# arkworks-rs/pcd

Hardware: NVIDIA B200
Metric: pcd_step_proofs_per_sec (higher is better)
Workload: dtype u32 (10x32-bit limbs, Montgomery, integer only)

## Files before the change

### pcd_b200/csrc/fp.cuh

```cuda
#pragma once
#include "constants.cuh"

#define FP_LIMBS 10

#if defined(__CUDACC__)
static __constant__ u32 pcd_modc_r4[FP_LIMBS + 2] = {
    ParamsR4::mod(0), ParamsR4::mod(1), ParamsR4::mod(2), ParamsR4::mod(3), ParamsR4::mod(4), ParamsR4::mod(5),
    ParamsR4::mod(6), ParamsR4::mod(7), ParamsR4::mod(8), ParamsR4::mod(9), ParamsR4::INV, 0};
#endif
template <class P>
PCD_HD u32 fp_mod_opaque(int i) {
#if defined(__CUDA_ARCH__)
  if (P::ID == 0) return pcd_modc_r4[i];
#endif
  return i < FP_LIMBS ? P::mod(i) : P::INV;
}

template <class P>
struct Fp {
  u32 l[FP_LIMBS];
  typedef P Params;
  static constexpr int WORDS = FP_LIMBS;

  PCD_HD static Fp zero() {
    Fp r;
#pragma unroll
    for (int i = 0; i < FP_LIMBS; i++) r.l[i] = 0;
    return r;
  }
  PCD_HD static Fp one() {
    Fp r;
#pragma unroll
    for (int i = 0; i < FP_LIMBS; i++) r.l[i] = P::one(i);
    return r;
  }
  PCD_HD static Fp r2() {
    Fp r;
#pragma unroll
    for (int i = 0; i < FP_LIMBS; i++) r.l[i] = P::r2(i);
    return r;
  }
  PCD_HD bool is_zero() const {
    u32 t = 0;
#pragma unroll
    for (int i = 0; i < FP_LIMBS; i++) t |= l[i];
    return t == 0;
  }
  PCD_HD bool operator==(const Fp& o) const {
    u32 t = 0;
#pragma unroll
    for (int i = 0; i < FP_LIMBS; i++) t |= l[i] ^ o.l[i];
    return t == 0;
  }
  PCD_HD bool operator!=(const Fp& o) const { return !(*this == o); }

  PCD_HD static void reduce_once(u32* a) {
    u32 t[FP_LIMBS];
    t[0] = prims::sub_cc(a[0], P::mod(0));
#pragma unroll
    for (int i = 1; i < FP_LIMBS; i++) t[i] = prims::subc_cc(a[i], P::mod(i));
    u32 borrow = prims::subc(0, 0);
#pragma unroll
    for (int i = 0; i < FP_LIMBS; i++) a[i] = borrow ? a[i] : t[i];
  }

  PCD_HD friend Fp operator+(const Fp& a, const Fp& b) {
    Fp r;
    r.l[0] = prims::add_cc(a.l[0], b.l[0]);
#pragma unroll
    for (int i = 1; i < FP_LIMBS - 1; i++) r.l[i] = prims::addc_cc(a.l[i], b.l[i]);
    r.l[FP_LIMBS - 1] = prims::addc(a.l[FP_LIMBS - 1], b.l[FP_LIMBS - 1]);
    reduce_once(r.l);
    return r;
  }
  PCD_HD friend Fp operator-(const Fp& a, const Fp& b) {
    Fp r;
    r.l[0] = prims::sub_cc(a.l[0], b.l[0]);
#pragma unroll
    for (int i = 1; i < FP_LIMBS; i++) r.l[i] = prims::subc_cc(a.l[i], b.l[i]);
    u32 borrow = prims::subc(0, 0);
    u32 t[FP_LIMBS];
    t[0] = prims::add_cc(r.l[0], P::mod(0));
#pragma unroll
    for (int i = 1; i < FP_LIMBS - 1; i++) t[i] = prims::addc_cc(r.l[i], P::mod(i));
    t[FP_LIMBS - 1] = prims::addc(r.l[FP_LIMBS - 1], P::mod(FP_LIMBS - 1));
#pragma unroll
    for (int i = 0; i < FP_LIMBS; i++) r.l[i] = borrow ? t[i] : r.l[i];
    return r;
  }
  PCD_HD Fp neg() const {
    if (is_zero()) return *this;
    Fp r;
    r.l[0] = prims::sub_cc(P::mod(0), l[0]);
#pragma unroll
    for (int i = 1; i < FP_LIMBS - 1; i++) r.l[i] = prims::subc_cc(P::mod(i), l[i]);
    r.l[FP_LIMBS - 1] = prims::subc(P::mod(FP_LIMBS - 1), l[FP_LIMBS - 1]);
    return r;
  }
  PCD_HD Fp dbl() const { return *this + *this; }

  PCD_HD static void mul_n(u32* acc, const u32* a, u32 bi, int n = FP_LIMBS) {
#pragma unroll
    for (int j = 0; j < n; j += 2) {
      acc[j] = prims::mul_lo(a[j], bi);
      acc[j + 1] = prims::mul_hi(a[j], bi);
    }
  }
  PCD_HD static void cmad_n(u32* acc, const u32* a, u32 bi, int n = FP_LIMBS) {
    acc[0] = prims::mad_lo_cc(a[0], bi, acc[0]);
    acc[1] = prims::madc_hi_cc(a[0], bi, acc[1]);
#pragma unroll
    for (int j = 2; j < n; j += 2) {
      acc[j] = prims::madc_lo_cc(a[j], bi, acc[j]);
      acc[j + 1] = prims::madc_hi_cc(a[j], bi, acc[j + 1]);
    }
  }
  template <int OFF>
  PCD_HD static void cmad_mod(u32* acc, u32 m) {
    acc[0] = prims::mad_lo_cc(fp_mod_opaque<P>(OFF), m, acc[0]);
    acc[1] = prims::madc_hi_cc(fp_mod_opaque<P>(OFF), m, acc[1]);
#pragma unroll
    for (int j = 2; j < FP_LIMBS; j += 2) {
      acc[j] = prims::madc_lo_cc(fp_mod_opaque<P>(OFF + j), m, acc[j]);
      acc[j + 1] = prims::madc_hi_cc(fp_mod_opaque<P>(OFF + j), m, acc[j + 1]);
    }
  }
  PCD_HD static void madc_n_rshift(u32* odd, const u32* a, u32 bi) {
#pragma unroll
    for (int j = 0; j < FP_LIMBS - 2; j += 2) {
      odd[j] = prims::madc_lo_cc(a[j], bi, odd[j + 2]);
      odd[j + 1] = prims::madc_hi_cc(a[j], bi, odd[j + 3]);
    }
    odd[FP_LIMBS - 2] = prims::madc_lo_cc(a[FP_LIMBS - 2], bi, 0);
    odd[FP_LIMBS - 1] = prims::madc_hi(a[FP_LIMBS - 2], bi, 0);
  }
  PCD_HD static void mont_row(u32* even, u32* odd, const u32* a, u32 bi, bool first) {
    if (first) {
      mul_n(odd, a + 1, bi);
      mul_n(even, a, bi);
    } else {
      even[0] = prims::add_cc(even[0], odd[1]);
      madc_n_rshift(odd, a + 1, bi);
      cmad_n(even, a, bi);
      odd[FP_LIMBS - 1] = prims::addc(odd[FP_LIMBS - 1], 0);
    }
    u32 m = prims::mul_lo(even[0], fp_mod_opaque<P>(FP_LIMBS));
    cmad_mod<1>(odd, m);
    cmad_mod<0>(even, m);
    odd[FP_LIMBS - 1] = prims::addc(odd[FP_LIMBS - 1], 0);
  }

  PCD_HD friend Fp operator*(const Fp& a, const Fp& b) {
    return mul_cc(a, b);
  }
  PCD_HD static Fp mul_cc(const Fp& a, const Fp& b) {
    u32 even[FP_LIMBS], odd[FP_LIMBS];
#pragma unroll
    for (int i = 0; i < FP_LIMBS; i += 2) {
      mont_row(even, odd, a.l, b.l[i], i == 0);
      mont_row(odd, even, a.l, b.l[i + 1], false);
    }
    Fp r;
    r.l[0] = prims::add_cc(even[0], odd[1]);
#pragma unroll
    for (int i = 1; i < FP_LIMBS - 1; i++) r.l[i] = prims::addc_cc(even[i], odd[i + 1]);
    r.l[FP_LIMBS - 1] = prims::addc(even[FP_LIMBS - 1], 0);
    reduce_once(r.l);
    return r;
  }
  PCD_HD Fp sqr() const { return (*this) * (*this); }
  PCD_NOINLINE static Fp mul_ni(Fp a, Fp b) { return a * b; }

  template <u32 K>
  PCD_HD Fp mul_small() const {
    static_assert(K >= 1 && K < 256, "small constant");
    Fp acc = *this;
    bool started = false;
    Fp r = *this;
#pragma unroll
    for (int bit = 7; bit >= 0; bit--) {
      if (started) r = r.dbl();
      if ((K >> bit) & 1) {
        if (started) r = r + acc;
        else started = true;
      }
    }
    return r;
  }

  PCD_HD static constexpr u32 pm2(int i) {
    u64 borrow = 2;
    u32 out = 0;
    for (int k = 0; k <= i; k++) {
      u64 v = P::mod(k);
      out = (u32)(v - borrow);
      borrow = (v < borrow) ? 1 : 0;
    }
    return out;
  }
  PCD_HD Fp inverse_fermat() const {
    Fp r = one();
    bool started = false;
    for (int i = FP_LIMBS - 1; i >= 0; i--) {
      u32 e = 0;
#pragma unroll
      for (int k = 0; k < FP_LIMBS; k++)
        if (k == i) e = pm2(k);
      for (int b = 31; b >= 0; b--) {
        if (started) r = r.sqr();
        if ((e >> b) & 1) {
          r = started ? r * (*this) : *this;
          started = true;
        }
      }
    }
    return r;
  }
  PCD_HD static void shr1(u32* a) {
#pragma unroll
    for (int i = 0; i < FP_LIMBS - 1; i++) a[i] = (a[i] >> 1) | (a[i + 1] << 31);
    a[FP_LIMBS - 1] >>= 1;
  }
  PCD_HD static void halve_mod(u32* x) {
    if (x[0] & 1) {
      x[0] = prims::add_cc(x[0], P::mod(0));
#pragma unroll
      for (int i = 1; i < FP_LIMBS - 1; i++) x[i] = prims::addc_cc(x[i], P::mod(i));
      x[FP_LIMBS - 1] = prims::addc(x[FP_LIMBS - 1], P::mod(FP_LIMBS - 1));
    }
    shr1(x);
  }
  PCD_HD static bool geq(const u32* a, const u32* b) {
    prims::sub_cc(a[0], b[0]);
#pragma unroll
    for (int i = 1; i < FP_LIMBS; i++) prims::subc_cc(a[i], b[i]);
    return prims::subc(0, 0) == 0;
  }
  PCD_HD static void sub_raw(u32* a, const u32* b) {
    a[0] = prims::sub_cc(a[0], b[0]);
#pragma unroll
    for (int i = 1; i < FP_LIMBS - 1; i++) a[i] = prims::subc_cc(a[i], b[i]);
    a[FP_LIMBS - 1] = prims::subc(a[FP_LIMBS - 1], b[FP_LIMBS - 1]);
  }
  PCD_HD static bool is_one_raw(const u32* a) {
    u32 t = a[0] ^ 1u;
#pragma unroll
    for (int i = 1; i < FP_LIMBS; i++) t |= a[i];
    return t == 0;
  }
  PCD_HD Fp inverse() const {
    if (is_zero()) return *this;
    u32 u[FP_LIMBS], v[FP_LIMBS];
    Fp x1 = zero(), x2 = zero();
    x1.l[0] = 1;
#pragma unroll
    for (int i = 0; i < FP_LIMBS; i++) {
      u[i] = l[i];
      v[i] = P::mod(i);
    }
    while (!is_one_raw(u) && !is_one_raw(v)) {
      while (!(u[0] & 1)) {
        shr1(u);
        halve_mod(x1.l);
      }
      while (!(v[0] & 1)) {
        shr1(v);
        halve_mod(x2.l);
      }
      if (geq(u, v)) {
        sub_raw(u, v);
        x1 = x1 - x2;
      } else {
        sub_raw(v, u);
        x2 = x2 - x1;
      }
    }
    Fp r = is_one_raw(u) ? x1 : x2;
    return (r * r2()) * r2();
  }
  PCD_HD Fp pow64(u64 e) const {
    Fp r = one();
    Fp base = *this;
    while (e) {
      if (e & 1) r = r * base;
      e >>= 1;
      if (e) base = base.sqr();
    }
    return r;
  }
  PCD_HD Fp from_mont() const {
    Fp o = zero();
    o.l[0] = 1;
    return (*this) * o;
  }
  PCD_HD Fp to_mont() const { return (*this) * r2(); }
  PCD_HD static Fp from_u32(u32 v) {
    Fp o = zero();
    o.l[0] = v;
    return o.to_mont();
  }
  PCD_HD bool lexicographically_largest() const {
    Fp v = from_mont();
    Fp n = neg().from_mont();
#pragma unroll
    for (int i = FP_LIMBS - 1; i >= 0; i--) {
      if (v.l[i] != n.l[i]) return v.l[i] > n.l[i];
    }
    return false;
  }
};

typedef Fp<ParamsR4> FpR4;
typedef Fp<ParamsQ4> FpQ4;
```

### pcd_b200/csrc/msm.cuh

```cuda
#pragma once
#include <cstdlib>

#include <cub/device/device_radix_sort.cuh>
#include <cub/device/device_scan.cuh>

#include "common.cuh"
#include "vecio.cuh"
#include "wec.cuh"

static constexpr int MSM_SCALAR_BITS = 298;
static constexpr int MSM_HEAVY = 1024;
static constexpr int MSM_HEAVY_THREADS = 128;
static constexpr int MSM_MAX_HEAVY = 16384;
static constexpr int MSM_HEAVY_CHUNK = 1024;
static constexpr int MSM_REDUCE_LOGL = 3;
static constexpr int MSM_SUM_PER_GROUP = 4;
static constexpr int MSM_MAX_SPLIT = 4;

__host__ __device__ __forceinline__ int msm_win_start(int j, int c, int nwin, int balanced) {
  if (!balanced) return j * c;
  int base = (MSM_SCALAR_BITS + 1) / nwin, rem = (MSM_SCALAR_BITS + 1) % nwin;
  return j * base + (j < rem ? j : rem);
}

template <class SP>
__global__ void msm_digits_kernel(const u32* __restrict__ scalars, int mont, size_t n_main,
                                  const u32* __restrict__ extra, size_t n, int c, int nwin, int shared,
                                  int* __restrict__ dig, u32* __restrict__ counts, const uint4* __restrict__ bases,
                                  int point_u4, size_t base_first, u32 unit_k) {
  size_t i = (size_t)blockIdx.x * blockDim.x + threadIdx.x;
  if (i >= n) return;
  {
    const uint4* bp = bases + (base_first + i) * (size_t)point_u4;
    u32 any = 0;
    for (int q = 0; q < point_u4; q++) {
      uint4 v = __ldg(bp + q);
      any |= v.x | v.y | v.z | v.w;
    }
    if (any == 0) {
      for (int w = 0; w < nwin; w++) dig[(size_t)w * n + i] = 0;
      return;
    }
  }
  Fp<SP> k;
  const bool is_extra = i >= n_main;
  const uint2* p = reinterpret_cast<const uint2*>(is_extra ? extra + (i - n_main) * 10 : scalars + i * 10);
  if (is_extra) mont = 0;
#pragma unroll
  for (int j = 0; j < 5; j++) {
    uint2 v = __ldg(p + j);
    k.l[2 * j] = v.x;
    k.l[2 * j + 1] = v.y;
  }
  if (mont) k = k.from_mont();
  const u32 B = 1u << (c - 1);
  if (unit_k) {
    u32 rest = 0;
#pragma unroll
    for (int j = 1; j < 10; j++) rest |= k.l[j];
    if (rest == 0 && k.l[0] == 1u) {
      const u32 b = B + (u32)(i & (size_t)(unit_k - 1));
      dig[i] = (int)(b + 1);
      for (int w = 1; w < nwin; w++) dig[(size_t)w * n + i] = 0;
      atomicAdd(&counts[b], 1u);
      return;
    }
  }
  u32 w32[12];
#pragma unroll
  for (int j = 0; j < 10; j++) w32[j] = k.l[j];
  w32[10] = 0;
  w32[11] = 0;
  u32 carry = 0;
  for (int w = 0; w < nwin; w++) {
    int bit = msm_win_start(w, c, nwin, shared);
    int cw = (w + 1 < nwin ? msm_win_start(w + 1, c, nwin, shared) : (shared ? MSM_SCALAR_BITS + 1 : bit + c)) - bit;
    const u32 mask = (1u << cw) - 1;
    const u32 half = 1u << (cw - 1);
    int limb = bit >> 5, off = bit & 31;
    u32 d = 0;
    if (limb < 10) {
      unsigned long long v = w32[limb] | ((unsigned long long)w32[limb + 1] << 32);
      d = (u32)(v >> off) & mask;
    }
    d += carry;
    int sd;
    if (d > half) {
      sd = (int)d - (int)(1u << cw);
      carry = 1;
    } else {
      sd = (int)d;
      carry = 0;
    }
    dig[(size_t)w * n + i] = sd;
    if (sd != 0) {
      u32 b = (u32)(sd < 0 ? -sd : sd) - 1;
      atomicAdd(&counts[(shared ? 0 : (size_t)w * B) + b], 1u);
    }
  }
}

static __global__ void msm_scatter_kernel(const int* __restrict__ dig, size_t n, int c, int nwin, int shared, size_t stride,
                                   size_t offset, u32* __restrict__ cursor, u32* __restrict__ entries) {
  size_t t = (size_t)blockIdx.x * blockDim.x + threadIdx.x;
  if (t >= n * (size_t)nwin) return;
  int sd = dig[t];
  if (sd == 0) return;
  size_t w = t / n, i = t - w * n;
  const u32 B = 1u << (c - 1);
  u32 b = (u32)(sd < 0 ? -sd : sd) - 1;
  u32 pos = atomicAdd(&cursor[(shared ? 0 : w * B) + b], 1u);
  entries[pos] = (u32)(shared ? w * stride + offset + i : i) | (sd < 0 ? 0x80000000u : 0u);
}

static __global__ void msm_sizekey_kernel(const u32* __restrict__ counts, size_t nbuckets, u32* __restrict__ key,
                                          u32* __restrict__ id) {
  size_t g = (size_t)blockIdx.x * blockDim.x + threadIdx.x;
  if (g >= nbuckets) return;
  u32 c = counts[g];
  key[g] = c < 2047u ? c : 2047u;
  id[g] = (u32)g;
}

static __global__ void msm_prof_entries_kernel(const u32* __restrict__ heavy, const u32* __restrict__ offsets, size_t nbuckets,
                                               u32* __restrict__ out) {
  u32 nheavy = heavy[0] < (u32)MSM_MAX_HEAVY ? heavy[0] : (u32)MSM_MAX_HEAVY;
  u32 h = 0;
  for (u32 i = threadIdx.x; i < nheavy; i += 32) h += offsets[heavy[1 + i] + 1] - offsets[heavy[1 + i]];
  for (int d = 16; d > 0; d >>= 1) h += __shfl_xor_sync(0xffffffffu, h, d);
  if (threadIdx.x == 0) {
    out[0] = offsets[nbuckets] - h;
    out[1] = h;
  }
}

__device__ __forceinline__ u32 msm_dynamic_heavy_thr(u32 host_thr, u32 real_total, u32 resident_items, size_t nbuckets,
                                                     u32 split) {
  u32 share = real_total / (resident_items ? resident_items : 1u);
  u32 item = share / 2 > 8u ? share / 2 : 8u;
  u32 dyn = split * item;
  u32 floor_thr = 2u * (u32)(real_total / nbuckets) + 8u;
  if (dyn < floor_thr) dyn = floor_thr;
  if (dyn < 24u) dyn = 24u;
  return dyn < host_thr ? dyn : host_thr;
}

static __global__ void __launch_bounds__(1024) msm_plan_small_kernel(const u32* __restrict__ counts, u32 nbuckets,
                                                                      u32* __restrict__ offsets, u32* __restrict__ cursor,
                                                                      u32* __restrict__ perm, u32* __restrict__ heavy,
                                                                      u32* __restrict__ queue) {
  __shared__ u32 key[1024];
  __shared__ u32 warp_sum[32];
  const u32 t = threadIdx.x;
  const u32 c = t < nbuckets ? counts[t] : 0u;
  key[t] = c < 2047u ? c : 2047u;
  u32 v = c;
  for (int d = 1; d < 32; d <<= 1) {
    u32 o = __shfl_up_sync(0xffffffffu, v, d);
    if ((t & 31u) >= (u32)d) v += o;
  }
  if ((t & 31u) == 31u) warp_sum[t >> 5] = v;
  __syncthreads();
  if (t < 32) {
    u32 w = warp_sum[t];
    for (int d = 1; d < 32; d <<= 1) {
      u32 o = __shfl_up_sync(0xffffffffu, w, d);
      if (t >= (u32)d) w += o;
    }
    warp_sum[t] = w;
  }
  __syncthreads();
  const u32 incl = v + ((t >> 5) ? warp_sum[(t >> 5) - 1] : 0u);
  if (t < nbuckets) {
    offsets[t] = incl - c;
    cursor[t] = incl - c;
    if (t == nbuckets - 1) {
      offsets[nbuckets] = incl;
      cursor[nbuckets] = incl;
    }
    u32 rank = 0;
    const u32 mine = key[t];
    for (u32 j = 0; j < nbuckets; j++) {
      const u32 kj = key[j];
      rank += (kj > mine || (kj == mine && j < t)) ? 1u : 0u;
    }
    perm[rank] = t;
  }
  if (t == 0) {
    heavy[0] = 0;
    queue[0] = 0;
  }
}

template <class C, bool PRE>
__device__ __forceinline__ AffinePoint<typename C::F> ld_base(const void* bases, size_t idx) {
  return ld_vec<AffinePoint<typename C::F>>(bases, idx);
}

template <class C, bool PRE>
__global__ void __launch_bounds__(128) msm_accumulate_kernel(const void* __restrict__ bases,
                                                             const u32* __restrict__ offsets,
                                                             const u32* __restrict__ entries,
                                                             const u32* __restrict__ perm, size_t nbuckets,
                                                             void* __restrict__ buckets, u32* __restrict__ heavy,
                                                             u32* __restrict__ queue, u32 heavy_thr, u32 split,
                                                             u32* __restrict__ hflag, u32 quantum, u32 persistent_from,
                                                             u32 resident_items, u32 nweighted) {
  typedef typename C::F F;
  typedef C CF;
  typedef typename CF::F FF;
  const unsigned lane = threadIdx.x & 31;
  const size_t nitems = nbuckets * split;
  const bool may_retire = blockIdx.x < persistent_from;
  heavy_thr = msm_dynamic_heavy_thr(heavy_thr, offsets[nbuckets], resident_items, nbuckets, split);
  u32 walked = 0;
  for (;;) {
    if (may_retire && __shfl_sync(0xffffffffu, walked, 0) >= quantum) break;
    u32 first = 0;
    if (lane == 0) first = atomicAdd(queue, 32u);
    first = __shfl_sync(0xffffffffu, first, 0);
    if (first >= nitems) break;
    size_t t = (size_t)first + lane;
    if (t >= nitems) continue;
    const u32 part = (u32)(t % split);
    size_t g = perm[t / split];
    u32 lo = offsets[g], hi = offsets[g + 1];
    XYZZ<CF> acc = XYZZ<CF>::inf();
    if (hi - lo > heavy_thr && g < nweighted) {
      if (part != 0) continue;
      u32 slot = atomicAdd(&heavy[0], 1u);
      if (slot < (u32)MSM_MAX_HEAVY) {
        heavy[1 + slot] = (u32)g;
        hflag[g] = 0xffffffffu;
        continue;
      }
      if (split > 1) {
        for (u32 q = 1; q < split; q++) st_vec(buckets, g * split + q, acc);
      }
    } else if (split > 1) {
      const u32 len = hi - lo;
      const u32 a = lo + (u32)(((unsigned long long)len * part) / split);
      hi = lo + (u32)(((unsigned long long)len * (part + 1)) / split);
      lo = a;
    }
    walked += hi - lo;
    for (u32 e = lo; e < hi; e++) {
      u32 ent = entries[e];
      AffinePoint<FF> p = ld_base<C, PRE>(bases, ent & 0x7fffffffu);
      if (ent >> 31) p.y = p.y.neg();
      acc.madd_impl(p);
    }
    st_vec(buckets, g * split + part, acc);
  }
}
template <class CS>
__device__ __forceinline__ AffinePoint<typename CS::F> ld_base_sliced(const void* bases, size_t idx, int l) {
  AffinePoint<typename CS::F> p;
  const char* src = reinterpret_cast<const char*>(bases) + idx * (size_t)240;
  const uint2* px = reinterpret_cast<const uint2*>(src + 40 * l);
  const uint2* py = reinterpret_cast<const uint2*>(src + 120 + 40 * l);
#pragma unroll
  for (int i = 0; i < 5; i++) {
    uint2 a = __ldg(px + i), b = __ldg(py + i);
    p.x.c.l[2 * i] = a.x;
    p.x.c.l[2 * i + 1] = a.y;
    p.y.c.l[2 * i] = b.x;
    p.y.c.l[2 * i + 1] = b.y;
  }
  return p;
}
template <class CS>
__device__ __forceinline__ void st_xyzz_sliced(void* buckets, size_t idx, const XYZZ<CS>& a, int l) {
  char* dst = reinterpret_cast<char*>(buckets) + idx * (size_t)480 + 40 * l;
  const FpR4* co[4] = {&a.x.c, &a.y.c, &a.zz.c, &a.zzz.c};
#pragma unroll
  for (int q = 0; q < 4; q++) {
    uint2* d = reinterpret_cast<uint2*>(dst + 120 * q);
#pragma unroll
    for (int i = 0; i < 5; i++) d[i] = make_uint2(co[q]->l[2 * i], co[q]->l[2 * i + 1]);
  }
}
template <class CS>
__device__ __forceinline__ XYZZ<CS> ld_xyzz_sliced(const void* buckets, size_t idx, int l) {
  XYZZ<CS> a;
  const char* src = reinterpret_cast<const char*>(buckets) + idx * (size_t)480 + 40 * l;
  FpR4* co[4] = {&a.x.c, &a.y.c, &a.zz.c, &a.zzz.c};
#pragma unroll
  for (int q = 0; q < 4; q++) {
    const uint2* d = reinterpret_cast<const uint2*>(src + 120 * q);
#pragma unroll
    for (int i = 0; i < 5; i++) {
      uint2 v = d[i];
      co[q]->l[2 * i] = v.x;
      co[q]->l[2 * i + 1] = v.y;
    }
  }
  return a;
}

#ifndef PCD_SLICED_MIN_CTAS
#define PCD_SLICED_MIN_CTAS 3
#endif
template <class CS, bool PRE>
__global__ void __launch_bounds__(128, PCD_SLICED_MIN_CTAS) msm_accumulate_sliced_kernel(const void* __restrict__ bases,
                                                                    const u32* __restrict__ offsets,
                                                                    const u32* __restrict__ entries,
                                                                    const u32* __restrict__ perm, size_t nbuckets,
                                                                    void* __restrict__ buckets, u32* __restrict__ heavy,
                                                                    u32* __restrict__ queue, u32 heavy_thr, u32 split,
                                                                    u32* __restrict__ hflag, u32 quantum, u32 persistent_from,
                                                             u32 resident_items, u32 nweighted) {
  typedef typename CS::F FF;
  const unsigned lane = threadIdx.x & 31;
  const int l = (int)(lane % 3u);
  const unsigned grp = lane / 3u;
  const size_t nitems = nbuckets * split;
  const bool may_retire = blockIdx.x < persistent_from;
  heavy_thr = msm_dynamic_heavy_thr(heavy_thr, offsets[nbuckets], resident_items, nbuckets, split);
  u32 walked = 0;
  for (;;) {
    if (may_retire && __shfl_sync(0xffffffffu, walked, 0) >= quantum) break;
    u32 first = 0;
    if (lane == 0) first = atomicAdd(queue, 10u);
    first = __shfl_sync(0xffffffffu, first, 0);
    if (first >= nitems) break;
    if (grp >= 10) continue;
    size_t t = (size_t)first + grp;
    if (t >= nitems) continue;
    const u32 part = (u32)(t % split);
    size_t g = perm[t / split];
    u32 lo = offsets[g], hi = offsets[g + 1];
    XYZZ<CS> acc = XYZZ<CS>::inf();
    if (hi - lo > heavy_thr && g < nweighted) {
      if (part != 0) continue;
      u32 slot = 0;
      if (l == 0) slot = atomicAdd(&heavy[0], 1u);
      slot = __shfl_sync(FF::gmask(), slot, (int)(lane - l));
      if (slot < (u32)MSM_MAX_HEAVY) {
        if (l == 0) {
          heavy[1 + slot] = (u32)g;
          hflag[g] = 0xffffffffu;
        }
        continue;
      }
      if (split > 1) {
        for (u32 q = 1; q < split; q++) st_xyzz_sliced<CS>(buckets, g * split + q, acc, l);
      }
    } else if (split > 1) {
      const u32 len = hi - lo;
      const u32 a = lo + (u32)(((unsigned long long)len * part) / split);
      hi = lo + (u32)(((unsigned long long)len * (part + 1)) / split);
      lo = a;
    }
    walked += hi - lo;
    for (u32 e = lo; e < hi; e++) {
      u32 ent = entries[e];
      AffinePoint<FF> p = ld_base_sliced<CS>(bases, ent & 0x7fffffffu, l);
      if (ent >> 31) p.y = p.y.neg();
      acc.madd_impl(p);
    }
    st_xyzz_sliced<CS>(buckets, g * split + part, acc, l);
  }
}
template <class CS>
__global__ void __launch_bounds__(96) msm_fold_parts_sliced_kernel(const void* __restrict__ partials, size_t nbuckets, u32 split,
                                                                   const u32* __restrict__ hflag, void* __restrict__ buckets) {
  const unsigned lane = threadIdx.x & 31, warp = threadIdx.x >> 5;
  if (lane >= 30) return;
  const int l = (int)(lane % 3u);
  size_t g = ((size_t)blockIdx.x * 3 + warp) * 10 + lane / 3u;
  if (g >= nbuckets || hflag[g] == 0xffffffffu) return;
  XYZZ<CS> acc = ld_xyzz_sliced<CS>(partials, g * split, l);
  for (u32 q = 1; q < split; q++) acc.add_impl(ld_xyzz_sliced<CS>(partials, g * split + q, l));
  st_xyzz_sliced<CS>(buckets, g, acc, l);
}

template <class C>
__global__ void __launch_bounds__(128) msm_fold_parts_kernel(const void* __restrict__ partials, size_t nbuckets, u32 split,
                                                             const u32* __restrict__ hflag, void* __restrict__ buckets) {
  size_t g = (size_t)blockIdx.x * blockDim.x + threadIdx.x;
  if (g >= nbuckets || hflag[g] == 0xffffffffu) return;
  XYZZ<C> acc = ld_vec_rw<XYZZ<C>>(partials, g * split);
  for (u32 q = 1; q < split; q++) acc.add(ld_vec_rw<XYZZ<C>>(partials, g * split + q));
  st_vec(buckets, g, acc);
}

template <class C>
__device__ __forceinline__ void cta_tree_sum(XYZZ<C>* sm, const XYZZ<C>& mine) {
  typedef Wec<C> WG;
  constexpr int NG = MSM_HEAVY_THREADS / WG::G;
  sm[threadIdx.x] = mine;
  u32* pts = reinterpret_cast<u32*>(sm);
  WG wg(pts + (size_t)MSM_HEAVY_THREADS * WG::PW + (size_t)(threadIdx.x / WG::G) * WG::NTW);
  const int g = (int)threadIdx.x / WG::G;
  for (int s = MSM_HEAVY_THREADS / 2; s > 0; s >>= 1) {
    __syncthreads();
    for (int i = g; i < s; i += NG) wg.add(pts + (size_t)i * WG::PW, pts + (size_t)(i + s) * WG::PW);
  }
  __syncthreads();
}
template <class C>
constexpr size_t cta_tree_smem() {
  return (size_t)MSM_HEAVY_THREADS * sizeof(XYZZ<C>) + (size_t)(MSM_HEAVY_THREADS / Wec<C>::G) * Wec<C>::NTW * 4;
}

template <class C, bool PRE>
__global__ void __launch_bounds__(MSM_HEAVY_THREADS) msm_accumulate_heavy_kernel(
    const void* __restrict__ bases, const u32* __restrict__ offsets, const u32* __restrict__ entries,
    const u32* __restrict__ heavy, u32* __restrict__ hp_count, u32* __restrict__ hp_id, void* __restrict__ hp_sum) {
  typedef typename C::F F;
  extern __shared__ uint4 sm4[];
  XYZZ<C>* sm = reinterpret_cast<XYZZ<C>*>(sm4);
  u32 nheavy = heavy[0] < (u32)MSM_MAX_HEAVY ? heavy[0] : (u32)MSM_MAX_HEAVY;
  u32 job = 0;
  for (u32 h = 0; h < nheavy; h++) {
    u32 g = heavy[1 + h];
    u32 lo = offsets[g], hi = offsets[g + 1];
    u32 nchunks = (hi - lo + MSM_HEAVY_CHUNK - 1) / MSM_HEAVY_CHUNK;
    for (u32 ch = 0; ch < nchunks; ch++, job++) {
      if (job % gridDim.x != blockIdx.x) continue;
      u32 e0 = lo + ch * MSM_HEAVY_CHUNK;
      u32 e1 = e0 + MSM_HEAVY_CHUNK < hi ? e0 + MSM_HEAVY_CHUNK : hi;
      XYZZ<C> acc = XYZZ<C>::inf();
      for (u32 e = e0 + threadIdx.x; e < e1; e += MSM_HEAVY_THREADS) {
        u32 ent = entries[e];
        AffinePoint<typename C::F> p = ld_base<C, PRE>(bases, ent & 0x7fffffffu);
        if (ent >> 31) p.y = p.y.neg();
        acc.madd(p);
      }
      cta_tree_sum<C>(sm, acc);
      if (threadIdx.x == 0) {
        u32 slot = atomicAdd(hp_count, 1u);
        hp_id[slot] = h;
        st_vec(hp_sum, slot, sm[0]);
      }
      __syncthreads();
    }
  }
}
template <class C>
__global__ void __launch_bounds__(MSM_HEAVY_THREADS) msm_heavy_finish_kernel(
    const u32* __restrict__ heavy, const u32* __restrict__ hp_count, const u32* __restrict__ hp_id,
    const void* __restrict__ hp_sum, void* __restrict__ buckets) {
  extern __shared__ uint4 sm4[];
  XYZZ<C>* sm = reinterpret_cast<XYZZ<C>*>(sm4);
  u32 nheavy = heavy[0] < (u32)MSM_MAX_HEAVY ? heavy[0] : (u32)MSM_MAX_HEAVY;
  u32 np = *hp_count;
  for (u32 h = blockIdx.x; h < nheavy; h += gridDim.x) {
    XYZZ<C> acc = XYZZ<C>::inf();
    for (u32 s = threadIdx.x; s < np; s += MSM_HEAVY_THREADS)
      if (hp_id[s] == h) acc.add(ld_vec_rw<XYZZ<C>>(hp_sum, s));
    cta_tree_sum<C>(sm, acc);
    if (threadIdx.x == 0) st_vec(buckets, heavy[1 + h], sm[0]);
    __syncthreads();
  }
}

static constexpr int MSM_HEAVY_CHUNK_SLICED = 320;
static constexpr int MSM_HEAVY_GROUPS = 40;
template <class CS>
__device__ __noinline__ XYZZ<CS> sliced_add_ni(XYZZ<CS> a, XYZZ<CS> b) {
  a.add_impl(b);
  return a;
}
template <class CS>
__device__ __noinline__ XYZZ<CS> sliced_madd_ni(XYZZ<CS> a, AffinePoint<typename CS::F> p) {
  a.madd_impl(p);
  return a;
}
template <class CS>
__device__ __forceinline__ void cta_tree_sum_sliced(void* sm, XYZZ<CS>& acc, int G, int l, bool live) {
  if (live) st_xyzz_sliced<CS>(sm, (size_t)G, acc, l);
  __syncthreads();
  for (int s = 32; s > 0; s >>= 1) {
    if (live && G < s && G + s < MSM_HEAVY_GROUPS) {
      acc = sliced_add_ni<CS>(acc, ld_xyzz_sliced<CS>(sm, (size_t)(G + s), l));
      st_xyzz_sliced<CS>(sm, (size_t)G, acc, l);
    }
    __syncthreads();
  }
}
template <class CS, bool PRE>
__global__ void __launch_bounds__(128) msm_accumulate_heavy_sliced_kernel(
    const void* __restrict__ bases, const u32* __restrict__ offsets, const u32* __restrict__ entries,
    const u32* __restrict__ heavy, u32* __restrict__ hp_count, u32* __restrict__ hp_id, void* __restrict__ hp_sum) {
  typedef typename CS::F FF;
  extern __shared__ uint4 sm4[];
  const unsigned lane = threadIdx.x & 31, warp = threadIdx.x >> 5;
  const bool live = lane < 30;
  const int l = (int)(lane % 3u);
  const int G = (int)(warp * 10 + lane / 3u);
  u32 nheavy = heavy[0] < (u32)MSM_MAX_HEAVY ? heavy[0] : (u32)MSM_MAX_HEAVY;
  u32 job = 0;
  for (u32 h = 0; h < nheavy; h++) {
    u32 g = heavy[1 + h];
    u32 lo = offsets[g], hi = offsets[g + 1];
    u32 nchunks = (hi - lo + MSM_HEAVY_CHUNK_SLICED - 1) / MSM_HEAVY_CHUNK_SLICED;
    for (u32 ch = 0; ch < nchunks; ch++, job++) {
      if (job % gridDim.x != blockIdx.x) continue;
      u32 e0 = lo + ch * MSM_HEAVY_CHUNK_SLICED;
      u32 e1 = e0 + MSM_HEAVY_CHUNK_SLICED < hi ? e0 + MSM_HEAVY_CHUNK_SLICED : hi;
      XYZZ<CS> acc = XYZZ<CS>::inf();
      if (live) {
        for (u32 e = e0 + (u32)G; e < e1; e += MSM_HEAVY_GROUPS) {
          u32 ent = entries[e];
          AffinePoint<FF> p = ld_base_sliced<CS>(bases, ent & 0x7fffffffu, l);
          if (ent >> 31) p.y = p.y.neg();
          acc = sliced_madd_ni<CS>(acc, p);
        }
      }
      cta_tree_sum_sliced<CS>(sm4, acc, G, l, live);
      if (warp == 0 && lane < 3) {
        u32 slot = 0;
        if (lane == 0) {
          slot = atomicAdd(hp_count, 1u);
          hp_id[slot] = h;
        }
        slot = __shfl_sync(7u, slot, 0);
        st_xyzz_sliced<CS>(hp_sum, slot, acc, l);
      }
      __syncthreads();
    }
  }
}
template <class CS>
__global__ void __launch_bounds__(128) msm_heavy_finish_sliced_kernel(
    const u32* __restrict__ heavy, const u32* __restrict__ hp_count, const u32* __restrict__ hp_id,
    const void* __restrict__ hp_sum, void* __restrict__ buckets) {
  extern __shared__ uint4 sm4[];
  const unsigned lane = threadIdx.x & 31, warp = threadIdx.x >> 5;
  const bool live = lane < 30;
  const int l = (int)(lane % 3u);
  const int G = (int)(warp * 10 + lane / 3u);
  u32 nheavy = heavy[0] < (u32)MSM_MAX_HEAVY ? heavy[0] : (u32)MSM_MAX_HEAVY;
  u32 np = *hp_count;
  for (u32 h = blockIdx.x; h < nheavy; h += gridDim.x) {
    XYZZ<CS> acc = XYZZ<CS>::inf();
    if (live)
      for (u32 s = (u32)G; s < np; s += MSM_HEAVY_GROUPS)
        if (hp_id[s] == h) acc = sliced_add_ni<CS>(acc, ld_xyzz_sliced<CS>(hp_sum, s, l));
    cta_tree_sum_sliced<CS>(sm4, acc, G, l, live);
    if (warp == 0 && lane < 3) st_xyzz_sliced<CS>(buckets, heavy[1 + h], acc, l);
    __syncthreads();
  }
}


template <class C>
__global__ void xyzz_to_affine_kernel(const void* __restrict__ in, size_t n, void* __restrict__ out) {
  size_t i = (size_t)blockIdx.x * blockDim.x + threadIdx.x;
  if (i >= n) return;
  XYZZ<C> p = ld_vec_rw<XYZZ<C>>(in, i);
  st_vec(out, i, p.to_affine());
}

template <class C>
__global__ void fixed_table_kernel(const void* __restrict__ base, void* __restrict__ table) {
  typedef typename C::F F;
  int j = blockIdx.x * blockDim.x + threadIdx.x;
  if (j >= 75) return;
  AffinePoint<F> b = ld_vec<AffinePoint<F>>(base, 0);
  XYZZ<C> p = XYZZ<C>::from_affine(b);
  for (int i = 0; i < 4 * j; i++) p = p.dbl();
  AffinePoint<F> pj = p.to_affine();
  XYZZ<C> acc = XYZZ<C>::inf();
  for (int d = 1; d <= 15; d++) {
    acc.madd(pj);
    st_vec(table, (size_t)j * 15 + (d - 1), acc.to_affine());
  }
}
template <class C>
__global__ void __launch_bounds__(128) fixed_mul_kernel(const void* __restrict__ table,
                                                        const u32* __restrict__ scalars, size_t n,
                                                        void* __restrict__ out) {
  typedef typename C::F F;
  size_t i = (size_t)blockIdx.x * blockDim.x + threadIdx.x;
  if (i >= n) return;
  u32 k[10];
  const uint2* p = reinterpret_cast<const uint2*>(scalars + i * 10);
#pragma unroll
  for (int j = 0; j < 5; j++) {
    uint2 v = __ldg(p + j);
    k[2 * j] = v.x;
    k[2 * j + 1] = v.y;
  }
  XYZZ<C> acc = XYZZ<C>::inf();
  for (int j = 0; j < 75; j++) {
    u32 d = (k[j >> 3] >> ((j & 7) * 4)) & 15u;
    if (d) acc.madd(ld_vec<AffinePoint<F>>(table, (size_t)j * 15 + (d - 1)));
  }
  st_vec(out, i, acc.to_affine());
}

template <class C>
__global__ void __launch_bounds__(128) precompute_kernel(const void* __restrict__ bases, size_t n, int c, int nwin,
                                                         void* __restrict__ pre) {
  typedef typename C::F F;
  size_t i = (size_t)blockIdx.x * blockDim.x + threadIdx.x;
  if (i >= n) return;
  AffinePoint<F> a = ld_vec_rw<AffinePoint<F>>(bases, i);
  st_vec(pre, i, a);
  XYZZ<C> p = XYZZ<C>::from_affine(a);
  for (int j = 1; j < nwin; j++) {
    int nd = msm_win_start(j, c, nwin, 1) - msm_win_start(j - 1, c, nwin, 1);
    for (int b = 0; b < nd; b++) p = p.dbl();
    a = p.to_affine();
    st_vec(pre, (size_t)j * n + i, a);
    p = XYZZ<C>::from_affine(a);
  }
}

template <class C> struct MsmSliced { static constexpr bool value = false; typedef C type; };
#if defined(__CUDACC__)
template <> struct MsmSliced<CurveMnt6G2> { static constexpr bool value = true; typedef CurveMnt6G2S type; };
#endif
struct MsmPlan {
  int c, nwin, shared;
  size_t stride, offset;
};

template <class C>
static int msm_run(pcdgpu_ctx* ctx, const void* d_bases, const void* d_scalars, int scalars_mont, size_t n_main,
                   const void* d_extra, size_t n_extra, MsmPlan plan, void* d_out) {
  const size_t n = n_main + n_extra;
  typedef typename C::ScalarParams SP;
  cudaStream_t st = ctx->cur();
  if (n == 0) {
    PCD_CUDA(ctx, cudaMemsetAsync(d_out, 0, sizeof(XYZZ<C>), st));
    return 0;
  }
  const int c = plan.c, nwin = plan.nwin, shared = plan.shared;
  if ((size_t)nwin * (shared ? plan.stride : n) >= ((size_t)1 << 31)) {
    ctx->set_error("MSM of %zu points x %d windows exceeds the 31-bit entry index", n, nwin);
    return PCDGPU_E_ARG;
  }
  const size_t B = (size_t)1 << (c - 1);
  const int rwin = shared ? 1 : nwin;
  static const bool no_units = getenv("PCDGPU_NO_UNIT_BUCKETS") != nullptr;
  size_t unit_k = 0;
  if (shared && n >= ((size_t)1 << 14) && !no_units) {
    unit_k = 64;
    while (unit_k < (n >> 8) && unit_k < 16384) unit_k <<= 1;
  }
  const size_t nbuckets = (shared ? B : B * nwin) + unit_k;
  void *dig, *ent, *cnt, *bkt, *seg, *cub_tmp;
  PCD_TRY(ctx->scratch(SLOT_MSM_DIG, (size_t)nwin * n * 4, &dig));
  PCD_TRY(ctx->scratch(SLOT_MSM_ENT, (size_t)nwin * n * 4, &ent));
  size_t cstride = (nbuckets + 1 + 3) & ~(size_t)3;
  PCD_TRY(ctx->scratch(SLOT_MSM_CNT, (7 * cstride + MSM_MAX_HEAVY + 8) * 4, &cnt));
  u32* counts = (u32*)cnt;
  u32* offsets = counts + cstride;
  u32* cursor = offsets + cstride;
  u32* key_in = cursor + cstride;
  u32* key_out = key_in + cstride;
  u32* id_in = key_out + cstride;
  u32* perm = id_in + cstride;
  u32* heavy = perm + cstride;
  const bool small_plan = nbuckets <= 1024;
  PCD_CUDA(ctx, cudaMemsetAsync(counts, 0, cstride * 4, st));
  u32* queue = heavy + MSM_MAX_HEAVY + 2;
  if (!small_plan) {
    PCD_CUDA(ctx, cudaMemsetAsync(heavy, 0, 4, st));
    PCD_CUDA(ctx, cudaMemsetAsync(queue, 0, 4, st));
  }
  const int acc_slot = n < ((size_t)1 << 14) ? PROF_MSM_ACC_SMALL
                       : (sizeof(typename C::F) > 80 ? PROF_MSM_ACC_G2Q3
                                                     : (sizeof(typename C::F) > 40 ? PROF_MSM_ACC_G2 : PROF_MSM_ACC_G1));
  int ps = ctx->prof_begin(PROF_MSM_SORT, (double)n * nwin);
  ctx->launches += 5 + 2;
  msm_digits_kernel<SP><<<(unsigned)((n + 127) / 128), 128, 0, st>>>((const u32*)d_scalars, scalars_mont, n_main,
                                                                    (const u32*)d_extra, n, c, nwin,
                                                                    shared, (int*)dig, counts, (const uint4*)d_bases,
                                                                    (int)(sizeof(AffinePoint<typename C::F>) / 16),
                                                                    shared ? plan.offset : (size_t)0, (u32)unit_k);
  PCD_CUDA(ctx, cudaGetLastError());
  if (small_plan) {
    msm_plan_small_kernel<<<1, 1024, 0, st>>>(counts, (u32)nbuckets, offsets, cursor, perm, heavy, queue);
    PCD_CUDA(ctx, cudaGetLastError());
  } else {
  size_t cub_bytes = 0;
  cub::DeviceScan::ExclusiveSum(nullptr, cub_bytes, counts, offsets, (int)(nbuckets + 1), st);
  PCD_TRY(ctx->scratch(SLOT_CUB, cub_bytes + 16, &cub_tmp));
  PCD_CUDA(ctx, cub::DeviceScan::ExclusiveSum(cub_tmp, cub_bytes, counts, offsets, (int)(nbuckets + 1), st));
  PCD_CUDA(ctx, cudaMemcpyAsync(cursor, offsets, (nbuckets + 1) * 4, cudaMemcpyDeviceToDevice, st));
  msm_sizekey_kernel<<<(unsigned)((nbuckets + 255) / 256), 256, 0, st>>>(counts, nbuckets, key_in, id_in);
  PCD_CUDA(ctx, cudaGetLastError());
  size_t sort_bytes = 0;
  cub::DeviceRadixSort::SortPairsDescending(nullptr, sort_bytes, key_in, key_out, id_in, perm, (int)nbuckets, 0, 11, st);
  void* sort_tmp;
  PCD_TRY(ctx->scratch(SLOT_CUB2, sort_bytes + 16, &sort_tmp));
  PCD_CUDA(ctx, cub::DeviceRadixSort::SortPairsDescending(sort_tmp, sort_bytes, key_in, key_out, id_in, perm,
                                                          (int)nbuckets, 0, 11, st));
  ctx->launches += 4;
  }
  size_t total = (size_t)nwin * n;
  msm_scatter_kernel<<<(unsigned)((total + 255) / 256), 256, 0, st>>>((const int*)dig, n, c, nwin, shared,
                                                                      plan.stride, plan.offset, cursor, (u32*)ent);
  PCD_CUDA(ctx, cudaGetLastError());
  ctx->prof_end(ps);
  if (ctx->sort_done) {
    PCD_CUDA(ctx, cudaEventRecord(ctx->sort_done, st));
    ctx->sort_done = nullptr;
  }
  for (int gi = 0; gi < 3; gi++)
    if (ctx->gate_wait[gi]) {
      PCD_CUDA(ctx, cudaStreamWaitEvent(st, ctx->gate_wait[gi], 0));
      ctx->gate_wait[gi] = nullptr;
    }
  ps = ctx->prof_begin(acc_slot, (double)n * nwin);
  constexpr bool SLICED = MsmSliced<C>::value;
  constexpr size_t ITEMS_PER_CTA = SLICED ? 40 : 128;
  static int occ_cache[2][16] = {{0}};
  static bool attr_done[16] = {false};
  const int dev_slot = ctx->device & 15;
  int acc_ctas = occ_cache[shared ? 1 : 0][dev_slot];
  if (acc_ctas == 0) {
  if constexpr (SLICED) {
    if (shared) PCD_CUDA(ctx, cudaOccupancyMaxActiveBlocksPerMultiprocessor(&acc_ctas, msm_accumulate_sliced_kernel<typename MsmSliced<C>::type, true>, 128, 0));
    else PCD_CUDA(ctx, cudaOccupancyMaxActiveBlocksPerMultiprocessor(&acc_ctas, msm_accumulate_sliced_kernel<typename MsmSliced<C>::type, false>, 128, 0));
  } else {
    if (shared) PCD_CUDA(ctx, cudaOccupancyMaxActiveBlocksPerMultiprocessor(&acc_ctas, msm_accumulate_kernel<C, true>, 128, 0));
    else PCD_CUDA(ctx, cudaOccupancyMaxActiveBlocksPerMultiprocessor(&acc_ctas, msm_accumulate_kernel<C, false>, 128, 0));
  }
  if (acc_ctas < 1) acc_ctas = 1;
  occ_cache[shared ? 1 : 0][dev_slot] = acc_ctas;
  }
  static const int acc_cap_env = getenv("PCDGPU_ACC_CTAS") ? atoi(getenv("PCDGPU_ACC_CTAS")) : 0;
  const int acc_cap = acc_cap_env > 0 ? acc_cap_env : (SLICED ? 4 : (ctx->concurrent && ctx->in_proof ? 2 : 3));
  if (acc_ctas > acc_cap) acc_ctas = acc_cap;
  size_t acc_grid = (size_t)acc_ctas * ctx->sm_count;
  size_t avg_entries = total / nbuckets;
  u32 heavy_thr = (u32)(4 * avg_entries < 64 ? 64 : (4 * avg_entries > (size_t)MSM_HEAVY ? (size_t)MSM_HEAVY : 4 * avg_entries));
  {
    size_t resident = acc_grid * 128;
    size_t even = 4 * (total / (resident ? resident : 1)) + 32;
    if (nbuckets * 8 < resident && even < heavy_thr) heavy_thr = (u32)even;
  }
  u32 split = 1;
  static const int split_env = getenv("PCDGPU_ACC_SPLIT") ? atoi(getenv("PCDGPU_ACC_SPLIT")) : 0;
  const u32 max_split = split_env > 0 ? (u32)split_env : (u32)MSM_MAX_SPLIT;
  while (split < max_split && nbuckets * split < 6 * acc_grid * ITEMS_PER_CTA && avg_entries / (2 * split) >= 8) split *= 2;
  if (split_env <= 0 && split == (u32)MSM_MAX_SPLIT && nbuckets * split < 2 * acc_grid * ITEMS_PER_CTA &&
      avg_entries / (4 * split) >= 8)
    split *= 2;
  if (acc_grid > (nbuckets * split + ITEMS_PER_CTA - 1) / ITEMS_PER_CTA) acc_grid = (nbuckets * split + ITEMS_PER_CTA - 1) / ITEMS_PER_CTA;
  static const int quantum_env = getenv("PCDGPU_ACC_QUANTUM") ? atoi(getenv("PCDGPU_ACC_QUANTUM")) : -1;
  u32 quantum = 0, persistent_from = 0;
  const u32 resident_items = (u32)(acc_grid * ITEMS_PER_CTA);
  {
    const int prods = SLICED ? 20 : (sizeof(typename C::F) / 40 == 1 ? 10 : 28);
    int q = quantum_env >= 0 ? quantum_env : (ctx->concurrent && ctx->in_proof ? 320 / prods : 0);
    if (q > 0) {
      const size_t resident = acc_grid;
      const size_t per_cta = (size_t)q * (SLICED ? 40 : 128);
      size_t extra = (total + per_cta - 1) / per_cta;
      if (extra > 65535) extra = 65535;
      quantum = (u32)q;
      persistent_from = (u32)extra;
      acc_grid = resident + extra;
    }
  }
  PCD_TRY(ctx->scratch(SLOT_MSM_BKT, nbuckets * sizeof(XYZZ<C>) * (split > 1 ? 1 + split : 1), &bkt));
  void* acc_out = split > 1 ? (void*)((char*)bkt + nbuckets * sizeof(XYZZ<C>)) : bkt;
  if constexpr (SLICED) {
    if (shared)
      msm_accumulate_sliced_kernel<typename MsmSliced<C>::type, true><<<(unsigned)acc_grid, 128, 0, st>>>(
          d_bases, offsets, (const u32*)ent, perm, nbuckets, acc_out, heavy, queue, heavy_thr, split, cursor, quantum, persistent_from, resident_items, (u32)(nbuckets - unit_k));
    else
      msm_accumulate_sliced_kernel<typename MsmSliced<C>::type, false><<<(unsigned)acc_grid, 128, 0, st>>>(
          d_bases, offsets, (const u32*)ent, perm, nbuckets, acc_out, heavy, queue, heavy_thr, split, cursor, quantum, persistent_from, resident_items, (u32)(nbuckets - unit_k));
  } else {
    if (shared)
      msm_accumulate_kernel<C, true><<<(unsigned)acc_grid, 128, 0, st>>>(d_bases, offsets, (const u32*)ent, perm, nbuckets,
                                                                       acc_out, heavy, queue, heavy_thr, split, cursor, quantum, persistent_from, resident_items, (u32)(nbuckets - unit_k));
    else
      msm_accumulate_kernel<C, false><<<(unsigned)acc_grid, 128, 0, st>>>(d_bases, offsets, (const u32*)ent, perm, nbuckets,
                                                                        acc_out, heavy, queue, heavy_thr, split, cursor, quantum, persistent_from, resident_items, (u32)(nbuckets - unit_k));
  }
  PCD_CUDA(ctx, cudaGetLastError());
  if (ctx->gate_done) {
    PCD_CUDA(ctx, cudaEventRecord(ctx->gate_done, st));
    ctx->gate_done = nullptr;
  }
  if (ps >= 0 && acc_slot != PROF_MSM_ACC_SMALL) {
    ctx->prof_end(ps);
    const int ps_acc = ps;
    ps = ctx->prof_begin(PROF_MSM_ACC_TAIL, 0.0);
    if (ctx->prof_pinned) {
      u32* pe = queue + 2;
      msm_prof_entries_kernel<<<1, 32, 0, st>>>(heavy, offsets, nbuckets, pe);
      ctx->spans[ps_acc].units_pinned = ps_acc;
      cudaMemcpyAsync(ctx->prof_pinned + ps_acc, pe, 4, cudaMemcpyDeviceToHost, st);
      if (ps >= 0) {
        ctx->spans[ps].units_pinned = ps;
        cudaMemcpyAsync(ctx->prof_pinned + ps, pe + 1, 4, cudaMemcpyDeviceToHost, st);
      }
    }
  } else if (ps >= 0 && ctx->prof_pinned) {
    ctx->spans[ps].units_pinned = ps;
    cudaMemcpyAsync(ctx->prof_pinned + ps, offsets + nbuckets, 4, cudaMemcpyDeviceToHost, st);
  }
  if (split > 1) {
    if constexpr (SLICED)
      msm_fold_parts_sliced_kernel<typename MsmSliced<C>::type><<<(unsigned)((nbuckets + 29) / 30), 96, 0, st>>>(
          acc_out, nbuckets, split, cursor, bkt);
    else
      msm_fold_parts_kernel<C><<<(unsigned)((nbuckets + 127) / 128), 128, 0, st>>>(acc_out, nbuckets, split, cursor, bkt);
    PCD_CUDA(ctx, cudaGetLastError());
    ctx->launches += 1;
  }
  size_t heavy_smem = cta_tree_smem<C>();
  size_t hp_cap = total / (SLICED ? MSM_HEAVY_CHUNK_SLICED : MSM_HEAVY_CHUNK) + MSM_MAX_HEAVY + 8;
  void* hp;
  PCD_TRY(ctx->scratch(SLOT_MSM_HP, hp_cap * (sizeof(XYZZ<C>) + 4) + 64, &hp));
  u32* hp_count = (u32*)hp;
  u32* hp_id = hp_count + 4;
  void* hp_sum = (char*)hp + 64 + ((hp_cap * 4 + 63) & ~(size_t)63);
  PCD_CUDA(ctx, cudaMemsetAsync(hp_count, 0, 4, st));
  if constexpr (SLICED) {
    typedef typename MsmSliced<C>::type CS;
    const size_t sl_smem = MSM_HEAVY_GROUPS * sizeof(XYZZ<C>);
    if (shared)
      msm_accumulate_heavy_sliced_kernel<CS, true><<<ctx->sm_count * 4, 128, sl_smem, st>>>(
          d_bases, offsets, (const u32*)ent, heavy, hp_count, hp_id, hp_sum);
    else
      msm_accumulate_heavy_sliced_kernel<CS, false><<<ctx->sm_count * 4, 128, sl_smem, st>>>(
          d_bases, offsets, (const u32*)ent, heavy, hp_count, hp_id, hp_sum);
    PCD_CUDA(ctx, cudaGetLastError());
    msm_heavy_finish_sliced_kernel<CS><<<64, 128, sl_smem, st>>>(heavy, hp_count, hp_id, hp_sum, bkt);
  } else {
    if (!attr_done[dev_slot]) {
      PCD_CUDA(ctx, cudaFuncSetAttribute(msm_accumulate_heavy_kernel<C, true>, cudaFuncAttributeMaxDynamicSharedMemorySize,
                                         (int)heavy_smem));
      PCD_CUDA(ctx, cudaFuncSetAttribute(msm_accumulate_heavy_kernel<C, false>, cudaFuncAttributeMaxDynamicSharedMemorySize,
                                         (int)heavy_smem));
      PCD_CUDA(ctx, cudaFuncSetAttribute(msm_heavy_finish_kernel<C>, cudaFuncAttributeMaxDynamicSharedMemorySize,
                                         (int)heavy_smem));
    }
    if (shared)
      msm_accumulate_heavy_kernel<C, true><<<ctx->sm_count * 4, MSM_HEAVY_THREADS, heavy_smem, st>>>(
          d_bases, offsets, (const u32*)ent, heavy, hp_count, hp_id, hp_sum);
    else
      msm_accumulate_heavy_kernel<C, false><<<ctx->sm_count * 4, MSM_HEAVY_THREADS, heavy_smem, st>>>(
          d_bases, offsets, (const u32*)ent, heavy, hp_count, hp_id, hp_sum);
    PCD_CUDA(ctx, cudaGetLastError());
    msm_heavy_finish_kernel<C><<<64, MSM_HEAVY_THREADS, heavy_smem, st>>>(heavy, hp_count, hp_id, hp_sum, bkt);
  }
  PCD_CUDA(ctx, cudaGetLastError());
  ctx->prof_end(ps);
  ps = ctx->prof_begin(PROF_MSM_REDUCE, (double)nbuckets);
  typedef Wec<C> WG;
  static const int logL_env = getenv("PCDGPU_REDUCE_LOGL") ? atoi(getenv("PCDGPU_REDUCE_LOGL")) : 0;
  static const int logL_small_env = getenv("PCDGPU_REDUCE_LOGL_SMALL") ? atoi(getenv("PCDGPU_REDUCE_LOGL_SMALL")) : 0;
  const int logL = logL_env > 0 ? logL_env : (B <= 1024 ? (logL_small_env > 0 ? logL_small_env : 1) : MSM_REDUCE_LOGL);
  const size_t L = (size_t)1 << logL;
  if (unit_k % L != 0) {
    ctx->set_error("unit buckets (%zu) are not a multiple of the reduction's group size (%zu)", unit_k, L);
    return PCDGPU_E_ARG;
  }
  const size_t T = ((B + L - 1) >> logL) + (unit_k >> logL);
  const size_t GPC = WEC_THREADS / WG::G;
  const size_t ctas = (T + GPC - 1) / GPC;
  const size_t per_cta = GPC * MSM_SUM_PER_GROUP;
  const size_t pitch = (ctas + per_cta - 1) / per_cta + 1;
  const size_t PB = sizeof(XYZZ<C>);
  PCD_TRY(ctx->scratch(SLOT_MSM_SEG, ((size_t)rwin * ctas + 2 * rwin * pitch + rwin + 8) * PB, &seg));
  char* sp = (char*)seg;
  void* lvl[2] = {sp + (size_t)rwin * ctas * PB, sp + ((size_t)rwin * ctas + rwin * pitch) * PB};
  void* wsum = (char*)lvl[1] + (size_t)rwin * pitch * PB;
  void* fin = rwin == 1 ? d_out : wsum;
  const size_t red_smem = wec_smem_bytes<C>(WEC_THREADS, 4), sum_smem = wec_smem_bytes<C>(WEC_THREADS, 2);
  if (!attr_done[dev_slot]) {
    PCD_CUDA(ctx, cudaFuncSetAttribute(wec_reduce_kernel<C>, cudaFuncAttributeMaxDynamicSharedMemorySize, (int)red_smem));
    PCD_CUDA(ctx, cudaFuncSetAttribute(wec_sum_kernel<C>, cudaFuncAttributeMaxDynamicSharedMemorySize, (int)sum_smem));
    attr_done[dev_slot] = true;
  }
  wec_reduce_kernel<C><<<dim3((unsigned)ctas, (unsigned)rwin), WEC_THREADS, red_smem, st>>>(bkt, B, logL,
                                                                                         ctas == 1 ? fin : seg, unit_k);
  PCD_CUDA(ctx, cudaGetLastError());
  ctx->launches += 1;
  const void* in = seg;
  size_t in_pitch = ctas, count = ctas;
  int pp = 0;
  while (count > 1) {
    size_t nct = (count + per_cta - 1) / per_cta;
    void* out = nct == 1 ? fin : lvl[pp];
    size_t out_pitch = nct == 1 ? 1 : pitch;
    wec_sum_kernel<C><<<dim3((unsigned)nct, (unsigned)rwin), WEC_THREADS, sum_smem, st>>>(in, in_pitch, count, out, out_pitch,
                                                                                       MSM_SUM_PER_GROUP);
    PCD_CUDA(ctx, cudaGetLastError());
    ctx->launches += 1;
    in = out;
    in_pitch = out_pitch;
    count = nct;
    pp ^= 1;
  }
  ctx->prof_end(ps);
  if (rwin > 1) {
    ps = ctx->prof_begin(PROF_MSM_TAIL, (double)rwin);
    wec_combine_kernel<C><<<1, 32, 0, st>>>(wsum, c, rwin, d_out);
    PCD_CUDA(ctx, cudaGetLastError());
    ctx->launches += 1;
    ctx->prof_end(ps);
  }
  return 0;
}
```

Measured before the change: 80.35.

## Add dedicated Montgomery squaring and warp-shuffle tree fold of MSM partials

Adds a Montgomery squaring routine that reuses the symmetry of cross products: it pre-doubles limbs and skips the lower-triangle multiplies. It is used for every field except the ID-0 parameter set, which keeps mul_cc. The non-sliced MSM partial-fold kernel now gives each split part its own lane and combines them with a warp-shuffle butterfly reduction instead of a serial per-thread loop, and the env-controlled split is capped at 32. The shuffle moves a whole XYZZ point per step, which adds register pressure and redundant point additions across lanes.

Result: slower. 77.36, median of 6 (-3.7%).

```diff
diff --git a/pcd_b200/csrc/fp.cuh b/pcd_b200/csrc/fp.cuh
--- a/pcd_b200/csrc/fp.cuh
+++ b/pcd_b200/csrc/fp.cuh
@@ -168,7 +168,62 @@
     reduce_once(r.l);
     return r;
   }
-  PCD_HD Fp sqr() const { return (*this) * (*this); }
+  PCD_HD static void sqr_row(u32* even, u32* odd, const u32* b, u32 bi, int from) {
+    even[0] = prims::add_cc(even[0], odd[1]);
+#pragma unroll
+    for (int j = 0; j < FP_LIMBS - 2; j += 2) {
+      if (j + 1 < from) {
+        odd[j] = prims::addc_cc(odd[j + 2], 0);
+        odd[j + 1] = prims::addc_cc(odd[j + 3], 0);
+      } else {
+        odd[j] = prims::madc_lo_cc(b[j + 1], bi, odd[j + 2]);
+        odd[j + 1] = prims::madc_hi_cc(b[j + 1], bi, odd[j + 3]);
+      }
+    }
+    odd[FP_LIMBS - 2] = prims::madc_lo_cc(b[FP_LIMBS - 1], bi, 0);
+    odd[FP_LIMBS - 1] = prims::madc_hi(b[FP_LIMBS - 1], bi, 0);
+    bool started = false;
+#pragma unroll
+    for (int j = 0; j < FP_LIMBS; j += 2) {
+      if (j < from) continue;
+      even[j] = started ? prims::madc_lo_cc(b[j], bi, even[j]) : prims::mad_lo_cc(b[j], bi, even[j]);
+      even[j + 1] = prims::madc_hi_cc(b[j], bi, even[j + 1]);
+      started = true;
+    }
+    if (started) odd[FP_LIMBS - 1] = prims::addc(odd[FP_LIMBS - 1], 0);
+    u32 m = prims::mul_lo(even[0], fp_mod_opaque<P>(FP_LIMBS));
+    cmad_mod<1>(odd, m);
+    cmad_mod<0>(even, m);
+    odd[FP_LIMBS - 1] = prims::addc(odd[FP_LIMBS - 1], 0);
+  }
+  PCD_HD static void sqr_mult(u32* b, const u32* a, int i) {
+#pragma unroll
+    for (int k = 0; k < FP_LIMBS; k++)
+      b[k] = k == i ? a[k] : (k == i + 1 || k == 0 ? a[k] << 1 : (a[k] << 1) | (a[k - 1] >> 31));
+  }
+  PCD_HD static Fp sqr_cc(const Fp& a) {
+    u32 b[FP_LIMBS];
+    u32 even[FP_LIMBS], odd[FP_LIMBS];
+#pragma unroll
+    for (int i = 0; i < FP_LIMBS; i += 2) {
+      sqr_mult(b, a.l, i);
+      if (i == 0) mont_row(even, odd, b, a.l[0], true);
+      else sqr_row(even, odd, b, a.l[i], i);
+      sqr_mult(b, a.l, i + 1);
+      sqr_row(odd, even, b, a.l[i + 1], i + 1);
+    }
+    Fp r;
+    r.l[0] = prims::add_cc(even[0], odd[1]);
+#pragma unroll
+    for (int i = 1; i < FP_LIMBS - 1; i++) r.l[i] = prims::addc_cc(even[i], odd[i + 1]);
+    r.l[FP_LIMBS - 1] = prims::addc(even[FP_LIMBS - 1], 0);
+    reduce_once(r.l);
+    return r;
+  }
+  PCD_HD Fp sqr() const {
+    if constexpr (P::ID == 0) return mul_cc(*this, *this);
+    else return sqr_cc(*this);
+  }
   PCD_NOINLINE static Fp mul_ni(Fp a, Fp b) { return a * b; }
 
   template <u32 K>
diff --git a/pcd_b200/csrc/msm.cuh b/pcd_b200/csrc/msm.cuh
--- a/pcd_b200/csrc/msm.cuh
+++ b/pcd_b200/csrc/msm.cuh
@@ -377,12 +377,22 @@
 
 template <class C>
 __global__ void __launch_bounds__(128) msm_fold_parts_kernel(const void* __restrict__ partials, size_t nbuckets, u32 split,
-                                                             const u32* __restrict__ hflag, void* __restrict__ buckets) {
-  size_t g = (size_t)blockIdx.x * blockDim.x + threadIdx.x;
-  if (g >= nbuckets || hflag[g] == 0xffffffffu) return;
-  XYZZ<C> acc = ld_vec_rw<XYZZ<C>>(partials, g * split);
-  for (u32 q = 1; q < split; q++) acc.add(ld_vec_rw<XYZZ<C>>(partials, g * split + q));
-  st_vec(buckets, g, acc);
+                                                             u32 lanes, const u32* __restrict__ hflag,
+                                                             void* __restrict__ buckets) {
+  const size_t t = (size_t)blockIdx.x * blockDim.x + threadIdx.x;
+  const size_t g = t / lanes;
+  const u32 q = (u32)(t % lanes);
+  const bool live = g < nbuckets && hflag[g] != 0xffffffffu;
+  XYZZ<C> acc = live && q < split ? ld_vec_rw<XYZZ<C>>(partials, g * split + q) : XYZZ<C>::inf();
+  for (u32 s = 1; s < lanes; s <<= 1) {
+    XYZZ<C> o;
+    u32* ow = reinterpret_cast<u32*>(&o);
+    const u32* aw = reinterpret_cast<const u32*>(&acc);
+#pragma unroll
+    for (int i = 0; i < (int)(sizeof(XYZZ<C>) / 4); i++) ow[i] = __shfl_xor_sync(0xffffffffu, aw[i], (int)s);
+    if (live) acc.add(o);
+  }
+  if (live && q == 0) st_vec(buckets, g, acc);
 }
 
 template <class C>
@@ -738,7 +748,7 @@
   }
   u32 split = 1;
   static const int split_env = getenv("PCDGPU_ACC_SPLIT") ? atoi(getenv("PCDGPU_ACC_SPLIT")) : 0;
-  const u32 max_split = split_env > 0 ? (u32)split_env : (u32)MSM_MAX_SPLIT;
+  const u32 max_split = split_env > 0 ? (split_env < 32 ? (u32)split_env : 32u) : (u32)MSM_MAX_SPLIT;
   while (split < max_split && nbuckets * split < 6 * acc_grid * ITEMS_PER_CTA && avg_entries / (2 * split) >= 8) split *= 2;
   if (split_env <= 0 && split == (u32)MSM_MAX_SPLIT && nbuckets * split < 2 * acc_grid * ITEMS_PER_CTA &&
       avg_entries / (4 * split) >= 8)
@@ -804,8 +814,12 @@
     if constexpr (SLICED)
       msm_fold_parts_sliced_kernel<typename MsmSliced<C>::type><<<(unsigned)((nbuckets + 29) / 30), 96, 0, st>>>(
           acc_out, nbuckets, split, cursor, bkt);
-    else
-      msm_fold_parts_kernel<C><<<(unsigned)((nbuckets + 127) / 128), 128, 0, st>>>(acc_out, nbuckets, split, cursor, bkt);
+    else {
+      u32 lanes = 1;
+      while (lanes < split) lanes <<= 1;
+      msm_fold_parts_kernel<C><<<(unsigned)((nbuckets * lanes + 127) / 128), 128, 0, st>>>(acc_out, nbuckets, split, lanes,
+                                                                                            cursor, bkt);
+    }
     PCD_CUDA(ctx, cudaGetLastError());
     ctx->launches += 1;
   }
```
